# Gwzwpxz/HDSDP

Hardware: AMD Instinct MI355X
Metric: IPM iterations/sec (Schur build+factor+solve), n=2000 m=2000 dense SDP (higher is better)
Workload: dtype f64

## Files before the change

hdsdp_amd/build.py:

```python
import os
import shutil
import subprocess
import sys

PKG = os.path.dirname(os.path.abspath(__file__))
ROOT = os.path.dirname(PKG)
CSRC = os.path.join(PKG, "csrc")
LIB = os.path.join(PKG, "libhdsdp_mi355x.so")
SOURCES = ["gemm_f64.hip", "gemm_persist.hip", "chol.hip", "schur.hip", "lanczos.hip", "lu.hip", "small.hip", "bsparse.hip", "engine.hip", "probes.hip", "coeff.cpp", "sdpa.cpp", "alloc.cpp"]
HEADERS = sorted(f for f in os.listdir(CSRC) if f.endswith(".h")) + [os.path.join(ROOT, "include", "hdsdp_mi355x.h")]


def _stale(target, deps):
    if not os.path.exists(target):
        return True
    t = os.path.getmtime(target)
    return any(os.path.getmtime(d) > t for d in deps)


def build_library(force=False, verbose=True, diagnostics=False):
    srcs = [os.path.join(CSRC, s) for s in SOURCES]
    hdrs = [h if os.path.isabs(h) else os.path.join(CSRC, h) for h in HEADERS]
    lib = LIB.replace(".so", "_diag.so") if diagnostics else LIB
    if not force and not _stale(lib, srcs + hdrs):
# ... 30 lines not shown
```

hdsdp_amd/csrc/gemm_f64.hip:

```cpp
#include "gemm_tile.h"
#include "gemm_persist.h"
namespace {
struct TimedLaunch { hipEvent_t e0, e1; int role; double flops, issued; };
bool g_timing = false;
thread_local bool g_capturing = false;
std::vector<TimedLaunch> g_timed;
unsigned long long *g_dbg = nullptr;
int g_dbg_role = -1;
struct TileList {
    int2 *dev = nullptr;
    int n = 0;
};
std::mutex g_tl_mutex;
std::map<std::tuple<int, int, int, int, int, unsigned long long>, TileList> g_tl_cache;

int g_reserved_cus = 0;
struct PersistDev { int *ring = nullptr; unsigned seq = 0; int slots = 0; };
std::map<int, PersistDev> g_persist_dev;
constexpr int PERSIST_RING = 256;
int persist_counters(int **cnt, int *slots) {
    int dev = 0;
    HDM_HIP_CHECK(hipGetDevice(&dev));
    std::lock_guard<std::mutex> lk(g_tl_mutex);
    PersistDev &pd = g_persist_dev[dev];
// ... 23 lines not shown
    }
    std::vector<int2> h;
    for (const HdmTile &t : hdm_tile_list(gm, subset)) h.push_back(make_int2(t.tm, t.tn));
    TileList tl;
    tl.n = (int) h.size();
    HDM_HIP_CHECK(hdm_malloc((void **) &tl.dev, sizeof(int2) * std::max<size_t>(1, h.size())));
    HDM_HIP_CHECK(hdm_memcpy_h2d_sync(tl.dev, h.data(), sizeof(int2) * h.size()));
    g_tl_cache[key] = tl;
    out = tl;
    return 0;
}
}

static int launch_tiles(const HdmGemmArgs &args, int subset, hipStream_t stream);

static HdmTileGeom tile_geom(const HdmGemmArgs &a) {
    return {a.M, a.N, a.K, a.klimit, a.lower_only, a.tile_col_mask, a.role, a.epilogue == HDM_EPI_SLAB, a.batch, a.k_base, a.k_chunk,
            ((a.role == HDM_ROLE_CONG2 || a.role == HDM_ROLE_GENERIC) && a.A2) ? 2 : 1};
}

static double issued_mfma_flops(const HdmGemmArgs &a, int subset) {
    return (double) hdm_launch_mfmas(tile_geom(a), subset) * 2048.0 * ((a.epilogue == HDM_EPI_SLAB) ? 1.0 : (double) a.batch);
}

int hdm_launch_gemm(const HdmGemmArgs &args, hipStream_t stream) {
    if (args.M <= 0 || args.N <= 0 || args.batch <= 0) return 0;
    if ((args.M % 8) || (args.N % 8) || (args.K % HDM_BK)) {
        fprintf(stderr, "[hdsdp_mi355x] gemm: M,N must be multiples of 8 and K of 16 (M=%d N=%d K=%d)\n",
                args.M, args.N, args.K);
        return 1;
    }
    if (args.epilogue == HDM_EPI_SLAB && (args.k_chunk <= 0 || args.k_chunk % HDM_BK)) {
        fprintf(stderr, "[hdsdp_mi355x] gemm: bad k_chunk\n");
        return 1;
    }
    if (args.role == HDM_ROLE_CONG2) {
        const bool mirrored = args.A2 == args.B && args.B2 == args.A && args.lda2 == args.ldb && args.ldb2 == args.lda &&
                              args.strideA2 == args.strideB && args.strideB2 == args.strideA;
        if (!mirrored || !args.lower_only || args.epilogue != HDM_EPI_BLOCKED || args.klimit != HDM_KLIM_BY_N ||
            args.M != args.N || args.a_kmajor || args.b_kmajor) {
            fprintf(stderr, "[hdsdp_mi355x] gemm role 2 is lower(A B^T + B A^T), blocked output, K cut by the column tile: launch refused\n");
            return 1;
        }
    }
    if (args.role != HDM_ROLE_GENERIC) {
        const long lds_[4] = {args.lda, args.ldb, args.A2 ? args.lda2 : 0, args.B2 ? args.ldb2 : 0};
        for (long ld : lds_)
            if (ld < 0 || ld > (1L << 20)) {
                fprintf(stderr, "[hdsdp_mi355x] gemm role %d: leading dimension %ld is beyond what the scalar stager addresses: launch refused\n", args.role, ld);
                return 1;
            }
        const HdmTileGeom gm = tile_geom(args);
        struct { const double *p; long span; bool km; long ld, kblk, stride; int rows; const char *nm; } ops[4] = {
            {args.A, args.spanA, args.a_kmajor != 0, args.lda, args.a_kblk, args.strideA, args.M, "A"},
            {args.B, args.spanB, args.b_kmajor != 0, args.ldb, args.b_kblk, args.strideB, args.N, "B"},
            {args.A2, args.spanA2, args.a_kmajor != 0, args.lda2, (long) HDM_BK, args.strideA2, args.M, "A2"},
// ... 35 lines not shown
    if (d.dbg && !g_capturing && getenv("HDM_DBG_SYNC")) HDM_HIP_CHECK(hipDeviceSynchronize());
#endif
    int var = 64;
#ifdef HDM_DIAGNOSTICS
    static const int g_env_var = [] { const char *e = getenv("HDM_VAR"); return e ? atoi(e) : -1; }();
    if (g_env_var >= 0) var = g_env_var;
    if (var == 576 && args.role != HDM_ROLE_CONG2) var = 64;
    if (args.role == HDM_ROLE_CONG2) {
        static const int g_direct = [] { const char *e = getenv("HDM_CONG2_DIRECT"); return e ? atoi(e) : 0; }();
        const bool direct = g_direct && var == 64 && args.A2 && !args.a_kmajor && !args.b_kmajor &&
                            args.epilogue == HDM_EPI_BLOCKED && args.lower_only && args.klimit == HDM_KLIM_BY_N &&
                            args.A2 == args.B && args.B2 == args.A;
        if (direct) var = 320;
    }
#endif
    long nwg = (long) tl.n * (args.batch >= 8 ? ((args.batch + 7) & ~7) : args.batch);
    static const int g_persist = [] { const char *e = getenv("HDM_PERSIST"); return e ? atoi(e) : 1; }();
    int *cnt = nullptr;
    const bool persist = g_persist && args.role != HDM_ROLE_GENERIC && args.batch >= 8 && !g_capturing &&
                         hdm_persist_supported(args.a_kmajor != 0, args.b_kmajor != 0, args.role, var);
    if (!persist && (var == 320 || var == 576)) var = 64;
    if (persist) {
        int slots = 0;
        if (persist_counters(&cnt, &slots)) return 1;
        HDM_HIP_CHECK(hipMemsetAsync(cnt, 0, 8 * sizeof(int), stream));
        nwg = std::min<long>(nwg, slots);
    }
    dim3 grid((unsigned) nwg), block(256);
    hipEvent_t e0 = nullptr, e1 = nullptr;
    const bool timed = g_timing && !g_capturing;
// ... 7 lines not shown
    } else {
#define HDM_LAUNCH(AK, BK, R, V) hipLaunchKernelGGL((hdm_gemm_kernel<AK, BK, R, V>), grid, block, 0, stream, d)
#ifdef HDM_DIAGNOSTICS
#define HDM_LAUNCH_V(AK, BK, R)                                   \
    switch (var) {                                                \
        case 32: HDM_LAUNCH(AK, BK, R, 32); break;                \
        case 96: HDM_LAUNCH(AK, BK, R, 96); break;                \
        case 192: HDM_LAUNCH(AK, BK, R, 192); break;              \
        case 0: HDM_LAUNCH(AK, BK, R, 0); break;                  \
        default: HDM_LAUNCH(AK, BK, R, 64);                       \
    }
#else
#define HDM_LAUNCH_V(AK, BK, R) HDM_LAUNCH(AK, BK, R, 64)
#endif
        switch (args.role) {
            case HDM_ROLE_CONG1: HDM_LAUNCH_V(false, true, HDM_ROLE_CONG1); break;
            case HDM_ROLE_CONG2: HDM_LAUNCH_V(false, false, HDM_ROLE_CONG2); break;
            case HDM_ROLE_GRAM: HDM_LAUNCH_V(true, true, HDM_ROLE_GRAM); break;
            case HDM_ROLE_CONG2D: HDM_LAUNCH_V(false, false, HDM_ROLE_CONG2D); break;
            default:
                if (lay == 3) HDM_LAUNCH(true, true, HDM_ROLE_GENERIC, 0);
                else if (lay == 2) HDM_LAUNCH(true, false, HDM_ROLE_GENERIC, 0);
                else if (lay == 1) HDM_LAUNCH(false, true, HDM_ROLE_GENERIC, 0);
#ifdef HDM_DIAGNOSTICS
                else if (var == 32) HDM_LAUNCH(false, false, HDM_ROLE_GENERIC, 32);
#endif
                else HDM_LAUNCH(false, false, HDM_ROLE_GENERIC, 0);
        }
    }
#undef HDM_LAUNCH_V
#undef HDM_LAUNCH
    if (timed) {
// ... 33 lines not shown
```

hdsdp_amd/csrc/gemm_geom.h:

```cpp
#pragma once
#include <algorithm>
#include <utility>
#include <vector>

#if defined(__HIPCC__)
#define HDM_HD __host__ __device__ __attribute__((always_inline))
#else
#define HDM_HD
#endif

#define HDM_TILE 128
#define HDM_BK 16
#define HDM_SUB 16

enum HdmKLimit { HDM_KLIM_NONE = 0, HDM_KLIM_BY_M = 1, HDM_KLIM_BY_N = 2, HDM_KLIM_BAND = 3 };
enum HdmEpilogue {
    HDM_EPI_STORE = 0,
    HDM_EPI_BLOCKED = 1,
    HDM_EPI_SLAB = 2
};
enum HdmRole { HDM_ROLE_GENERIC = 0, HDM_ROLE_CONG1 = 1, HDM_ROLE_CONG2 = 2, HDM_ROLE_GRAM = 3, HDM_ROLE_CONG2D = 4, HDM_NROLES = 5 };

HDM_HD inline long hdm_sky_panel(int t, int n) { return 128L * ((long) t * n - 64L * t * (t - 1)); }
HDM_HD inline long hdm_sky_off(int i, int j, int n) {
// ... 4 lines not shown
    const int t = (n + 127) / 128 - 1;
    const long w = n - 128L * t;
    return hdm_sky_panel(t, n) + w * w;
}

struct HdmTileGeom {
    int M, N, K;
    int klimit;
    int lower_only;
    unsigned long long colmask;
    int role;
    int slab;
    int batch;
    long k_base, k_chunk;
    int npass;
};
struct HdmTile { int tm, tn; };
struct HdmKRange { long kbeg, kend; };

HDM_HD constexpr int hdm_ntiles(int x) { return (x + HDM_TILE - 1) / HDM_TILE; }
HDM_HD constexpr int hdm_valid_subrows(int M, int tm) { return (M - tm * HDM_TILE + 15) >> 4; }
HDM_HD constexpr int hdm_cell_rows(int rv) { return rv < 4 ? 4 : rv; }
HDM_HD constexpr bool hdm_colmask_honoured(int NT) { return NT <= 64; }
HDM_HD constexpr unsigned long long hdm_colmask_effective(unsigned long long mask, int NT) { return hdm_colmask_honoured(NT) ? mask : 0ULL; }

HDM_HD constexpr bool hdm_tile_selected(const HdmTileGeom &g, int tm, int tn) {
    const unsigned long long mask = hdm_colmask_effective(g.colmask, hdm_ntiles(g.N));
    return !((g.lower_only || g.klimit == HDM_KLIM_BAND) && tm < tn) && !(mask && !((mask >> tn) & 1ULL));
}
HDM_HD constexpr bool hdm_full_diag(int M, int tm, int tn) { return tm == tn && hdm_valid_subrows(M, tm) >= 8; }
// ... 66 lines not shown
constexpr HdmLive HDM_LIVE_CONG1_FIRST[HDM_KBLOCK_PAIRS] = {{0, 0, 0}, {0, 1, 0}, {0, 2, 0}, {0, 3, 0}};
constexpr HdmLive HDM_LIVE_CONG1_LAST[HDM_KBLOCK_PAIRS] = {{0, 3, 0}, {0, 3, 1}, {0, 3, 2}, {0, 3, 3}};

HDM_HD constexpr int hdm_live_per_kstep(HdmLive l) { return (l.jhi - l.jlo + 1) * (4 - l.ilo); }
HDM_HD constexpr long hdm_pair_mfmas(HdmLive l) { return 2L * 4 * 4 * hdm_live_per_kstep(l); }
constexpr long HDM_KBLOCK_MFMAS = HDM_KBLOCK_PAIRS * hdm_pair_mfmas(HDM_LIVE_FULL);
HDM_HD constexpr long hdm_block_mfmas(const HdmLive (&t)[HDM_KBLOCK_PAIRS]) {
    long s = 0;
    for (int p = 0; p < HDM_KBLOCK_PAIRS; ++p) s += hdm_pair_mfmas(t[p]);
    return s;
}
HDM_HD constexpr long hdm_even_stages(long nst) { return nst <= 0 ? 0 : ((nst + 1) / 2) * 2; }
constexpr int HDM_DIAG_CELLS = 36;
HDM_HD constexpr int hdm_diag_short_cells(int RV) { return RV * (RV + 1) / 2; }
HDM_HD constexpr int hdm_edge_cells(int RV) { return 8 * RV; }
HDM_HD constexpr long hdm_tile_mfmas(const HdmTileGeom &g, int tm, int tn, int z) {
    const long nst = hdm_tile_stages(g, tm, tn, z);
    if (g.role == HDM_ROLE_GENERIC) return hdm_pair_mfmas(HDM_LIVE_FULL) / 2 * nst;
    const HdmTileClass c = hdm_tile_class(g, tm, tn);
    switch (c.kind) {
        case HDM_CLS_DIAG_FULL: return 4L * HDM_DIAG_CELLS * hdm_even_stages(nst);
        case HDM_CLS_DIAG_SHORT: return 4L * hdm_diag_short_cells(c.RV) * hdm_even_stages(nst);
        case HDM_CLS_EDGE: return 4L * hdm_edge_cells(c.RV) * hdm_even_stages(nst);
        case HDM_CLS_SYMDIAG: return tn * HDM_KBLOCK_MFMAS + hdm_block_mfmas(HDM_LIVE_CONG2D_LAST);
        default: break;
    }
    if (g.role == HDM_ROLE_CONG2) return 2 * (tn * HDM_KBLOCK_MFMAS + hdm_block_mfmas(HDM_LIVE_CONG2_LAST));
    if (g.role == HDM_ROLE_CONG1)
        return hdm_block_mfmas(HDM_LIVE_CONG1_FIRST) + (tm - tn - 1) * HDM_KBLOCK_MFMAS + hdm_block_mfmas(HDM_LIVE_CONG1_LAST);
    return hdm_pair_mfmas(HDM_LIVE_FULL) / 2 * hdm_even_stages(nst);
}
inline long hdm_launch_mfmas(const HdmTileGeom &g, int subset) {
    long mf = 0;
    for (int z = 0; z < (g.slab ? g.batch : 1); ++z)
// ... 68 lines not shown
```

hdsdp_amd/csrc/gemm_persist.h:

```cpp
#pragma once
#include "gemm_tile.h"

bool hdm_persist_supported(bool a_kmajor, bool b_kmajor, int role, int variant);
int hdm_launch_persist(bool a_kmajor, bool b_kmajor, int role, int variant, dim3 grid, dim3 block, hipStream_t stream,
                       const HdmGemmDev &d, int *cnt);
```

hdsdp_amd/csrc/gemm_persist.hip:

```cpp
#include "gemm_persist.h"

template <bool AK, bool BK, int R, int V>
static int launch_p(dim3 grid, dim3 block, hipStream_t stream, const HdmGemmDev &d, int *cnt) {
    hipLaunchKernelGGL((hdm_gemm_persist_kernel<AK, BK, R, V>), grid, block, 0, stream, d, cnt);
    return 0;
}

bool hdm_persist_supported(bool a_kmajor, bool b_kmajor, int role, int variant) {
#ifdef HDM_DIAGNOSTICS
    const bool common = (variant == 64 || variant == 96 || variant == 192);
    const bool cong2_extra = (variant == 320 || variant == 576);
#else
    const bool common = (variant == 64), cong2_extra = false;
#endif
    if (role == HDM_ROLE_CONG1) return !a_kmajor && b_kmajor && common;
    if (role == HDM_ROLE_CONG2) return !a_kmajor && !b_kmajor && (common || cong2_extra);
    if (role == HDM_ROLE_GRAM) return a_kmajor && b_kmajor && common;
    if (role == HDM_ROLE_CONG2D) return !a_kmajor && !b_kmajor && common;
    return false;
}

int hdm_launch_persist(bool a_kmajor, bool b_kmajor, int role, int variant, dim3 grid, dim3 block, hipStream_t stream,
                       const HdmGemmDev &d, int *cnt) {
    if (role == HDM_ROLE_CONG1 && !a_kmajor && b_kmajor) {
        if (variant == 64) return launch_p<false, true, HDM_ROLE_CONG1, 64>(grid, block, stream, d, cnt);
#ifdef HDM_DIAGNOSTICS
        if (variant == 96) return launch_p<false, true, HDM_ROLE_CONG1, 96>(grid, block, stream, d, cnt);
        if (variant == 192) return launch_p<false, true, HDM_ROLE_CONG1, 192>(grid, block, stream, d, cnt);
#endif
    } else if (role == HDM_ROLE_CONG2 && !a_kmajor && !b_kmajor) {
        if (variant == 64) return launch_p<false, false, HDM_ROLE_CONG2, 64>(grid, block, stream, d, cnt);
#ifdef HDM_DIAGNOSTICS
        if (variant == 96) return launch_p<false, false, HDM_ROLE_CONG2, 96>(grid, block, stream, d, cnt);
        if (variant == 192) return launch_p<false, false, HDM_ROLE_CONG2, 192>(grid, block, stream, d, cnt);
        if (variant == 320) return launch_p<false, false, HDM_ROLE_CONG2, 320>(grid, block, stream, d, cnt);
        if (variant == 576) return launch_p<false, false, HDM_ROLE_CONG2, 576>(grid, block, stream, d, cnt);
#endif
    } else if (role == HDM_ROLE_CONG2D && !a_kmajor && !b_kmajor) {
        if (variant == 64) return launch_p<false, false, HDM_ROLE_CONG2D, 64>(grid, block, stream, d, cnt);
#ifdef HDM_DIAGNOSTICS
        if (variant == 96) return launch_p<false, false, HDM_ROLE_CONG2D, 96>(grid, block, stream, d, cnt);
        if (variant == 192) return launch_p<false, false, HDM_ROLE_CONG2D, 192>(grid, block, stream, d, cnt);
#endif
    } else if (role == HDM_ROLE_GRAM && a_kmajor && b_kmajor) {
        if (variant == 64) return launch_p<true, true, HDM_ROLE_GRAM, 64>(grid, block, stream, d, cnt);
// ... 10 lines not shown
```

hdsdp_amd/csrc/gemm_tile.h:

```cpp
#pragma once
#include "hdm_common.h"
#include <algorithm>
#include <map>
#include <mutex>
#include <tuple>
#include <vector>

#define LDM 144
#define LDK 18
#define STAGE_DOUBLES 2304

struct HdmGemmDev {
    HdmGemmArgs a;
    const int2 *tiles;
    int ntiles;
    unsigned long long *dbg;
};

template <bool KM, bool DUAL = true>
struct Stager {
    const double *p;
    long qstride;
    long kstep;
    unsigned okmask;
// ... 244 lines not shown

template <class T> constexpr bool cell_uses_row(int q) {
    for (int c = 0; c < T::NC; ++c) if (T::si[c] == q) return true;
    return false;
}
template <class T> constexpr bool cell_uses_col(int q) {
    for (int c = 0; c < T::NC; ++c) if (T::sj[c] == q) return true;
    return false;
}
template <class T> constexpr int cell_frag_count() {
    int k = 0;
    for (int q = 0; q < 8; ++q) k += (cell_uses_row<T>(q) ? 1 : 0) + (cell_uses_col<T>(q) ? 1 : 0);
    return k;
}

template <class T, bool AKM, bool BKM, class STA, class STB>
__device__ __forceinline__ void cell_tile(const HdmGemmArgs &a, STA &stA, STB &stB, hdm_lchar *sb,
                                          int nst, int tid, int z, int m0, int n0, int l15, int lq, int rv, int tri) {
    hdm_d4 acc[4][4];
#pragma unroll
    for (int c = 0; c < 16; ++c) acc[c >> 2][c & 3] = (hdm_d4){0.0, 0.0, 0.0, 0.0};
    hdm_u4 ra0, ra1, ra2, ra3, rb0, rb1, rb2, rb3;
    double fr0[8], fc0[8], fr1[8], fc1[8];
    constexpr int NC = T::NC;
    constexpr int NF = cell_frag_count<T>();
    const hdm_lchar *rdA = sb + rd_lane<AKM>(0, l15, lq);
    const hdm_lchar *rdB = sb + 2 * STAGE_DOUBLES * 8 + rd_lane<BKM>(0, l15, lq);
    hdm_lchar *wrA = sb + wr_lane<AKM>(tid);
    hdm_lchar *wrB = sb + 2 * STAGE_DOUBLES * 8 + wr_lane<BKM>(tid);
#define HDM_CLDF(FR, FC, CB, kk)                                                                            \
    _Pragma("unroll") for (int q = 0; q < 8; ++q) {                                                         \
        if (cell_uses_row<T>(q)) FR[q] = lds_ld(rdA + rd_off<AKM>(CB, q, kk));                              \
        if (cell_uses_col<T>(q)) FC[q] = lds_ld(rdB + rd_off<BKM>(CB, q, kk));                              \
    }
#define HDM_CMMA(FR, FC)                                                                                    \
    _Pragma("unroll") for (int c = 0; c < NC; ++c)                                                          \
        acc[c >> 2][c & 3] = __builtin_amdgcn_mfma_f64_16x16x4f64(FC[T::sj[c]], FR[T::si[c]], acc[c >> 2][c & 3], 0, 0, 0);
#define HDM_CSTAGE(CB)                                                                                      \
    {                                                                                                       \
        HDM_CLDF(fr1, fc1, CB, 4)                                                                           \
        HDM_CMMA(fr0, fc0)                                                                                  \
        HDM_CLDF(fr0, fc0, CB, 8)                                                                           \
        HDM_CMMA(fr1, fc1)                                                                                  \
        HDM_CLDF(fr1, fc1, CB, 12)                                                                          \
        st4(wrA, (CB) ^ 1, ra0, ra1, ra2, ra3); st4(wrB, (CB) ^ 1, rb0, rb1, rb2, rb3);                     \
        HDM_CMMA(fr0, fc0)                                                                                  \
        sgb_spread<NC, 0x100, NF>();                                                                        \
        sgb_spread<NC, 0x100, NF>();                                                                        \
        sgb_spread<NC / 2, 0x100, NF>();                                                                    \
        sgb_spread<NC - NC / 2, 0x200, 8>();                                                                \
        __builtin_amdgcn_sched_barrier(0);                                                                  \
        __syncthreads();                                                                                    \
        __builtin_amdgcn_sched_barrier(0);                                                                  \
        HDM_CLDF(fr0, fc0, (CB) ^ 1, 0)                                                                     \
        stA.load_counted(ra0, ra1, ra2, ra3); stB.load_counted(rb0, rb1, rb2, rb3);    \
        HDM_CMMA(fr1, fc1)                                                                                  \
        __builtin_amdgcn_sched_group_barrier(0x100, NF, 0);                                                 \
        sgb_spread<NC, 0x20, 8>();                                                                          \
        __builtin_amdgcn_sched_barrier(0);                                                                  \
    }
#define HDM_CLAST(CB)                                                                                       \
    {                                                                                                       \
        HDM_CLDF(fr1, fc1, CB, 4)                                                                           \
        HDM_CMMA(fr0, fc0)                                                                                  \
        HDM_CLDF(fr0, fc0, CB, 8)                                                                           \
        HDM_CMMA(fr1, fc1)                                                                                  \
        HDM_CLDF(fr1, fc1, CB, 12)                                                                          \
        HDM_CMMA(fr0, fc0)                                                                                  \
        HDM_CMMA(fr1, fc1)                                                                                  \
    }
    stA.remain = nst; stB.remain = nst;
    if (nst > 0) {
        stA.load_counted(ra0, ra1, ra2, ra3); stB.load_counted(rb0, rb1, rb2, rb3);
        st4(wrA, 0, ra0, ra1, ra2, ra3); st4(wrB, 0, rb0, rb1, rb2, rb3);
        stA.load_counted(ra0, ra1, ra2, ra3); stB.load_counted(rb0, rb1, rb2, rb3);
    }
    __syncthreads();
    if (nst > 0) {
        HDM_CLDF(fr0, fc0, 0, 0)
        const int npairs = (nst + 1) >> 1;
        for (int t = 0; t + 1 < npairs; ++t) { HDM_CSTAGE(0) HDM_CSTAGE(1) }
        HDM_CSTAGE(0) HDM_CLAST(1)
    }
#undef HDM_CLDF
#undef HDM_CMMA
#undef HDM_CSTAGE
#undef HDM_CLAST
    cell_epilogue<T>(a, z, m0, n0, l15, lq, rv, tri, acc);
}

template <int JLO>
__device__ __forceinline__ void cd_mma(hdm_d4 (&acc)[4][4], const double (&fa)[4], const double (&fb)[4]) {
#pragma unroll
    for (int j = JLO; j < 4; ++j)
#pragma unroll
        for (int i = 0; i < 4; ++i) acc[j][i] = __builtin_amdgcn_mfma_f64_16x16x4f64(fa[j], fb[i], acc[j][i], 0, 0, 0);
}

// ... 108 lines not shown

    const int kt0 = (int) (kbeg / HDM_BK), kt1 = (int) (kend / HDM_BK);
    constexpr bool symdiag = (ROLE == HDM_ROLE_CONG2D);
#define HDM_CELL_STAMP(KIND)                                                                        \
    if ((VAR & 32) && p.dbg && tid == 0) {                                                          \
        unsigned long long *d = p.dbg + (size_t) sidx * 8;                                    \
        d[0] = t_start; d[1] = t_start; d[2] = t_start; d[3] = __builtin_amdgcn_s_memtime();        \
        d[4] = __builtin_amdgcn_s_getreg((15 << 11) | (0 << 6) | 4);                                \
        d[5] = __builtin_amdgcn_s_getreg((3 << 11) | (0 << 6) | 20);                                \
        d[6] = (unsigned long long) (long long) -(KIND);                                            \
        d[7] = __builtin_amdgcn_s_memrealtime();                                                    \
    }

    if constexpr (ROLE != HDM_ROLE_GENERIC) {
    constexpr bool DUAL = (ROLE == HDM_ROLE_CONG2);
    SStager<AKM, DUAL> stA;
    SStager<BKM, DUAL> stB;
    long ldb = a.ldb;
    if (ROLE == HDM_ROLE_CONG1 && a.b_sky) {
        ldb = a.N - 128L * tn;
        B += hdm_sky_panel(tn, a.N) - 128L * tn * (ldb + 1);
    }
    stA.init(A, a.lda, a.a_kblk, a.seg_rows, a.seg_extra, (VAR & 128) ? 0 : m0, kt0, tid, wave);
    stB.init(B, ldb, a.b_kblk, a.seg_rows, a.seg_extra, (VAR & 128) ? 0 : n0, kt0, tid, wave);
    int npass = 1;
    if constexpr (DUAL) {
        if (a.A2) {
            npass = 2;
            stA.chain(a.A2 + (long) z * a.strideA2, a.lda2, m0, kt0, wave, kt1 - kt0);
            stB.chain(a.B2 + (long) z * a.strideB2, a.ldb2, n0, kt0, wave, kt1 - kt0);
        }
    }
    if (!symdiag && a.lower_only && tm == tn) {
        const int nst = (kt1 - kt0) * npass;
        const int rvd = (a.M - m0 + 15) >> 4;
        if (rvd < 8) {
#define HDM_DEDGE(RV)                                                                                                      \
    switch (wave) {                                                                                                        \
        case 0: cell_tile<DiagEdgeCells<0, RV>, AKM, BKM>(a, stA, stB, sb, nst, tid, z, m0, n0, l15, lq, rvd, 1); break;  \
        case 1: cell_tile<DiagEdgeCells<1, RV>, AKM, BKM>(a, stA, stB, sb, nst, tid, z, m0, n0, l15, lq, rvd, 1); break;  \
        case 2: cell_tile<DiagEdgeCells<2, RV>, AKM, BKM>(a, stA, stB, sb, nst, tid, z, m0, n0, l15, lq, rvd, 1); break;  \
        default: cell_tile<DiagEdgeCells<3, RV>, AKM, BKM>(a, stA, stB, sb, nst, tid, z, m0, n0, l15, lq, rvd, 1); break; \
    }
            if (rvd <= 4) { HDM_DEDGE(4) } else if (rvd == 5) { HDM_DEDGE(5) } else if (rvd == 6) { HDM_DEDGE(6) } else { HDM_DEDGE(7) }
#undef HDM_DEDGE
            HDM_CELL_STAMP(3)
            return;
        }
        if constexpr (ROLE != HDM_ROLE_CONG2) {
            switch (wave) {
                case 0: cell_tile<DiagCells<0>, AKM, BKM>(a, stA, stB, sb, nst, tid, z, m0, n0, l15, lq, 8, 1); break;
                case 1: cell_tile<DiagCells<1>, AKM, BKM>(a, stA, stB, sb, nst, tid, z, m0, n0, l15, lq, 8, 1); break;
                case 2: cell_tile<DiagCells<2>, AKM, BKM>(a, stA, stB, sb, nst, tid, z, m0, n0, l15, lq, 8, 1); break;
                default: cell_tile<DiagCells<3>, AKM, BKM>(a, stA, stB, sb, nst, tid, z, m0, n0, l15, lq, 8, 1); break;
            }
            HDM_CELL_STAMP(1)
        }
        return;
    }
    if (!symdiag && tm != tn && m0 + HDM_TILE > a.M && n0 + HDM_TILE <= a.N) {
        const int nst = (kt1 - kt0) * npass;
        const int rv = (a.M - m0 + 15) >> 4;
#define HDM_EDGE(RV)                                                                                                     \
    switch (wave) {                                                                                                      \
        case 0: cell_tile<EdgeCells<0, RV>, AKM, BKM>(a, stA, stB, sb, nst, tid, z, m0, n0, l15, lq, rv, 0); break;  \
        case 1: cell_tile<EdgeCells<1, RV>, AKM, BKM>(a, stA, stB, sb, nst, tid, z, m0, n0, l15, lq, rv, 0); break;  \
        case 2: cell_tile<EdgeCells<2, RV>, AKM, BKM>(a, stA, stB, sb, nst, tid, z, m0, n0, l15, lq, rv, 0); break;  \
        default: cell_tile<EdgeCells<3, RV>, AKM, BKM>(a, stA, stB, sb, nst, tid, z, m0, n0, l15, lq, rv, 0); break; \
    }
        if (rv <= 4) { HDM_EDGE(4) } else if (rv == 5) { HDM_EDGE(5) } else if (rv == 6) { HDM_EDGE(6) } else { HDM_EDGE(7) }
#undef HDM_EDGE
        HDM_CELL_STAMP(2)
        return;
    }

    if constexpr (ROLE == HDM_ROLE_CONG2 && (VAR & 256) != 0) {
        cong2_direct_body(a, z, tm, tn, wm, wn, l15, lq);
        return;
    }
    {
        hdm_u4 ra0, ra1, ra2, ra3, rb0, rb1, rb2, rb3;
        const int nst = (kt1 - kt0) * npass;
        double fa0[4], fb0[4], fa1[4], fb1[4];
        const hdm_lchar *rdA = sb + rd_lane<AKM>(wm * 16, l15, lq);
        const hdm_lchar *rdB = sb + 2 * STAGE_DOUBLES * 8 + rd_lane<BKM>(wn * 16, l15, lq);
        hdm_lchar *wrA = sb + wr_lane<AKM>(tid);
        hdm_lchar *wrB = sb + 2 * STAGE_DOUBLES * 8 + wr_lane<BKM>(tid);
#define HDM_LDF(FA, FB, CB, kk)                                                                   \
    _Pragma("unroll") for (int i = 0; i < 4; ++i) FB[i] = lds_ld(rdA + rd_off<AKM>(CB, 2 * i, kk)); \
// ... 295 lines not shown
    const int x = (int) __builtin_amdgcn_s_getreg((3 << 11) | (0 << 6) | 20) & 7;
    const bool one_queue = (ROLE == HDM_ROLE_GRAM) && p.a.queue_global != 0;
    for (int dx = 0; dx < (one_queue ? 1 : 8); ++dx) {
        const int xq = one_queue ? 0 : ((x + dx) & 7);
        while (true) {
            __syncthreads();
            if (threadIdx.x == 0) s_idx = atomicAdd(&cnt[xq], 1);
            __syncthreads();
            const int idx = __builtin_amdgcn_readfirstlane(s_idx);
            const int z = one_queue ? idx / ntiles : xq + 8 * (idx / ntiles);
            if (z >= nb) break;
            hdm_gemm_tile<AKM, BKM, ROLE, VAR>(p, z, idx % ntiles, (long) z * ntiles + idx % ntiles);
        }
    }
}
```

Baseline: 2.858.

## Skip dead MFMA cells per K stage in CONG1/CONG2 diagonal and edge tiles

Adds an exact-liveness mode, on by default through HDM_EXACT_LIVE, for the CONG1 and CONG2 roles. Diagonal and edge cell tiles unroll their first and last K blocks with compile-time masks, so MFMAs whose sub-tile contributes only zeros at a given stage are not issued. The CONG2 edge path also uses unmasked loads. The old pair-live path is kept as a separate kernel variant in a new source file for when the mode is turned off. This trims wasted matrix-core work on triangular and banded tiles, at the cost of more template instantiations, larger code, and possible register pressure.

New measurement: 2.870 (median of 6 runs). Within noise of the previous version (+0.4%).

```diff
diff --git a/hdsdp_amd/build.py b/hdsdp_amd/build.py
--- a/hdsdp_amd/build.py
+++ b/hdsdp_amd/build.py
@@ -7,7 +7,7 @@
 ROOT = os.path.dirname(PKG)
 CSRC = os.path.join(PKG, "csrc")
 LIB = os.path.join(PKG, "libhdsdp_mi355x.so")
-SOURCES = ["gemm_f64.hip", "gemm_persist.hip", "chol.hip", "schur.hip", "lanczos.hip", "lu.hip", "small.hip", "bsparse.hip", "engine.hip", "probes.hip", "coeff.cpp", "sdpa.cpp", "alloc.cpp"]
+SOURCES = ["gemm_f64.hip", "gemm_persist.hip", "gemm_pairlive.hip", "chol.hip", "schur.hip", "lanczos.hip", "lu.hip", "small.hip", "bsparse.hip", "engine.hip", "probes.hip", "coeff.cpp", "sdpa.cpp", "alloc.cpp"]
 HEADERS = sorted(f for f in os.listdir(CSRC) if f.endswith(".h")) + [os.path.join(ROOT, "include", "hdsdp_mi355x.h")]
 
 
diff --git a/hdsdp_amd/csrc/gemm_f64.hip b/hdsdp_amd/csrc/gemm_f64.hip
--- a/hdsdp_amd/csrc/gemm_f64.hip
+++ b/hdsdp_amd/csrc/gemm_f64.hip
@@ -61,9 +61,15 @@
 
 static int launch_tiles(const HdmGemmArgs &args, int subset, hipStream_t stream);
 
+static bool exact_live() {
+    static const int g_exact = [] { const char *e = getenv("HDM_EXACT_LIVE"); return e ? atoi(e) : 1; }();
+    return g_exact != 0;
+}
+
 static HdmTileGeom tile_geom(const HdmGemmArgs &a) {
     return {a.M, a.N, a.K, a.klimit, a.lower_only, a.tile_col_mask, a.role, a.epilogue == HDM_EPI_SLAB, a.batch, a.k_base, a.k_chunk,
-            ((a.role == HDM_ROLE_CONG2 || a.role == HDM_ROLE_GENERIC) && a.A2) ? 2 : 1};
+            ((a.role == HDM_ROLE_CONG2 || a.role == HDM_ROLE_GENERIC) && a.A2) ? 2 : 1,
+            ((a.role == HDM_ROLE_CONG1 || a.role == HDM_ROLE_CONG2) && exact_live()) ? (HDM_EXACT_CELLS | HDM_EXACT_CELLS2) : 0};
 }
 
 static double issued_mfma_flops(const HdmGemmArgs &a, int subset) {
@@ -87,6 +93,13 @@
         if (!mirrored || !args.lower_only || args.epilogue != HDM_EPI_BLOCKED || args.klimit != HDM_KLIM_BY_N ||
             args.M != args.N || args.a_kmajor || args.b_kmajor) {
             fprintf(stderr, "[hdsdp_mi355x] gemm role 2 is lower(A B^T + B A^T), blocked output, K cut by the column tile: launch refused\n");
+            return 1;
+        }
+    }
+    if (args.role == HDM_ROLE_CONG1) {
+        if (args.klimit != HDM_KLIM_BAND || !args.lower_only || args.M != args.N || args.M != args.K || args.epilogue == HDM_EPI_SLAB ||
+            args.a_kmajor || !args.b_kmajor || args.A2 || args.B2) {
+            fprintf(stderr, "[hdsdp_mi355x] gemm role 1 is lower(A B^T) over the K band of a square launch, A M-major, B K-major: launch refused\n");
             return 1;
         }
     }
@@ -152,6 +165,7 @@
         if (direct) var = 320;
     }
 #endif
+    if (var == 64 && !exact_live() && (args.role == HDM_ROLE_CONG1 || args.role == HDM_ROLE_CONG2)) var = 64 | HDM_VAR_PAIR_LIVE;
     long nwg = (long) tl.n * (args.batch >= 8 ? ((args.batch + 7) & ~7) : args.batch);
     static const int g_persist = [] { const char *e = getenv("HDM_PERSIST"); return e ? atoi(e) : 1; }();
     int *cnt = nullptr;
@@ -189,8 +203,14 @@
 #define HDM_LAUNCH_V(AK, BK, R) HDM_LAUNCH(AK, BK, R, 64)
 #endif
         switch (args.role) {
-            case HDM_ROLE_CONG1: HDM_LAUNCH_V(false, true, HDM_ROLE_CONG1); break;
-            case HDM_ROLE_CONG2: HDM_LAUNCH_V(false, false, HDM_ROLE_CONG2); break;
+            case HDM_ROLE_CONG1:
+                if (var == (64 | HDM_VAR_PAIR_LIVE)) { if (hdm_launch_pairlive(args.role, grid, block, stream, d, nullptr)) return 1; }
+                else HDM_LAUNCH_V(false, true, HDM_ROLE_CONG1);
+                break;
+            case HDM_ROLE_CONG2:
+                if (var == (64 | HDM_VAR_PAIR_LIVE)) { if (hdm_launch_pairlive(args.role, grid, block, stream, d, nullptr)) return 1; }
+                else HDM_LAUNCH_V(false, false, HDM_ROLE_CONG2);
+                break;
             case HDM_ROLE_GRAM: HDM_LAUNCH_V(true, true, HDM_ROLE_GRAM); break;
             case HDM_ROLE_CONG2D: HDM_LAUNCH_V(false, false, HDM_ROLE_CONG2D); break;
             default:
diff --git a/hdsdp_amd/csrc/gemm_geom.h b/hdsdp_amd/csrc/gemm_geom.h
--- a/hdsdp_amd/csrc/gemm_geom.h
+++ b/hdsdp_amd/csrc/gemm_geom.h
@@ -42,6 +42,7 @@
     int batch;
     long k_base, k_chunk;
     int npass;
+    int exact_live;
 };
 struct HdmTile { int tm, tn; };
 struct HdmKRange { long kbeg, kend; };
@@ -138,10 +139,85 @@
 constexpr int HDM_DIAG_CELLS = 36;
 HDM_HD constexpr int hdm_diag_short_cells(int RV) { return RV * (RV + 1) / 2; }
 HDM_HD constexpr int hdm_edge_cells(int RV) { return 8 * RV; }
+
+enum HdmZeroRule {
+    HDM_Z_NONE = 0,
+    HDM_Z_COLS_UPTO = 1,
+    HDM_Z_ROWS_FROM = 2,
+    HDM_Z_COLS_FROM = 4
+};
+constexpr int HDM_Z_CONG1_FIRST = HDM_Z_COLS_UPTO, HDM_Z_CONG1_LAST = HDM_Z_ROWS_FROM;
+constexpr int HDM_Z_CONG1_DIAG = HDM_Z_COLS_UPTO | HDM_Z_ROWS_FROM;
+constexpr int HDM_Z_CONG2_LAST = HDM_Z_COLS_FROM;
+constexpr int HDM_Z_CONG2D_LAST = HDM_Z_ROWS_FROM | HDM_Z_COLS_FROM;
+constexpr int HDM_KBLOCK_STAGES = HDM_TILE / HDM_BK;
+HDM_HD constexpr bool hdm_subtile_live(int rules, int s, int si, int sj) {
+    return !((rules & HDM_Z_COLS_UPTO) && sj > s) && !((rules & HDM_Z_ROWS_FROM) && si < s) && !((rules & HDM_Z_COLS_FROM) && sj < s);
+}
+HDM_HD constexpr HdmLive hdm_live_exact(int rules, int s, int wm, int wn) {
+    return {(rules & HDM_Z_COLS_FROM) ? (s - wn + 1) / 2 : 0, (rules & HDM_Z_COLS_UPTO) ? (s - wn + 2) / 2 - 1 : 3,
+            (rules & HDM_Z_ROWS_FROM) ? (s - wm + 1) / 2 : 0};
+}
+HDM_HD constexpr long hdm_block_mfmas_exact(int rules) {
+    long mf = 0;
+    for (int s = 0; s < HDM_KBLOCK_STAGES; ++s)
+        for (int w = 0; w < 4; ++w) mf += 4L * hdm_live_per_kstep(hdm_live_exact(rules, s, w & 1, w >> 1));
+    return mf;
+}
+struct HdmStageRange { int lo, hi; };
+HDM_HD constexpr HdmStageRange hdm_cell_stage_range(int rules, int si, int sj) {
+    const int hi_r = (rules & HDM_Z_ROWS_FROM) ? si : HDM_KBLOCK_STAGES - 1, hi_c = (rules & HDM_Z_COLS_FROM) ? sj : HDM_KBLOCK_STAGES - 1;
+    return {(rules & HDM_Z_COLS_UPTO) ? sj : 0, hi_r < hi_c ? hi_r : hi_c};
+}
+HDM_HD constexpr int hdm_cells_live(HdmTileKind kind, int RV, int rules, int s) {
+    int n = 0;
+    for (int si = 0; si < (kind == HDM_CLS_DIAG_FULL ? 8 : RV); ++si)
+        for (int sj = 0; sj < (kind == HDM_CLS_EDGE ? 8 : si + 1); ++sj) {
+            const HdmStageRange r = hdm_cell_stage_range(rules, si, sj);
+            n += (r.lo <= s && s <= r.hi) ? 1 : 0;
+        }
+    return n;
+}
+HDM_HD constexpr long hdm_cell_block_mfmas(HdmTileKind kind, int RV, int rules, int nstages) {
+    long mf = 0;
+    for (int s = 0; s < nstages; ++s) mf += 4L * hdm_cells_live(kind, RV, rules, s);
+    return mf;
+}
+enum HdmExactLive { HDM_EXACT_CELLS = 1, HDM_EXACT_MAIN = 2, HDM_EXACT_CELLS2 = 4 };
+HDM_HD constexpr int hdm_exact_stages(int RV) { return RV >= 8 ? 8 : (RV + 1) / 2 * 2; }
+HDM_HD constexpr long hdm_tile_mfmas_exact(const HdmTileGeom &g, const HdmTileClass &c, int tm, int tn) {
+    const bool cells = (g.exact_live & HDM_EXACT_CELLS) != 0, mains = (g.exact_live & HDM_EXACT_MAIN) != 0;
+    if (g.role == HDM_ROLE_CONG1) {
+        if (c.kind == HDM_CLS_DIAG_FULL || c.kind == HDM_CLS_DIAG_SHORT)
+            return cells ? hdm_cell_block_mfmas(c.kind, c.RV, HDM_Z_CONG1_DIAG, c.RV) : -1;
+        if (c.kind == HDM_CLS_EDGE)
+            return cells ? hdm_cell_block_mfmas(c.kind, c.RV, HDM_Z_CONG1_FIRST, HDM_KBLOCK_STAGES) +
+                               (tm - tn - 1) * 4L * hdm_edge_cells(c.RV) * HDM_KBLOCK_STAGES +
+                               hdm_cell_block_mfmas(c.kind, c.RV, HDM_Z_CONG1_LAST, c.RV)
+                         : -1;
+        return mains ? hdm_block_mfmas_exact(HDM_Z_CONG1_FIRST) + (tm - tn - 1) * HDM_KBLOCK_MFMAS + hdm_block_mfmas_exact(HDM_Z_CONG1_LAST) : -1;
+    }
+    if (g.role == HDM_ROLE_CONG2) {
+        if (c.kind == HDM_CLS_EDGE)
+            return (g.exact_live & HDM_EXACT_CELLS2) ? 2 * (tn * 4L * hdm_edge_cells(c.RV) * HDM_KBLOCK_STAGES +
+                                hdm_cell_block_mfmas(c.kind, c.RV, HDM_Z_CONG2_LAST, HDM_KBLOCK_STAGES))
+                         : -1;
+        if (c.kind == HDM_CLS_MAIN) return mains ? 2 * (tn * HDM_KBLOCK_MFMAS + hdm_block_mfmas_exact(HDM_Z_CONG2_LAST)) : -1;
+        return -1;
+    }
+    if (g.role == HDM_ROLE_CONG2D && c.kind == HDM_CLS_SYMDIAG)
+        return mains ? tn * HDM_KBLOCK_MFMAS + hdm_block_mfmas_exact(HDM_Z_CONG2D_LAST) : -1;
+    return -1;
+}
+
 HDM_HD constexpr long hdm_tile_mfmas(const HdmTileGeom &g, int tm, int tn, int z) {
     const long nst = hdm_tile_stages(g, tm, tn, z);
     if (g.role == HDM_ROLE_GENERIC) return hdm_pair_mfmas(HDM_LIVE_FULL) / 2 * nst;
     const HdmTileClass c = hdm_tile_class(g, tm, tn);
+    if (g.exact_live) {
+        const long mf = hdm_tile_mfmas_exact(g, c, tm, tn);
+        if (mf >= 0) return mf;
+    }
     switch (c.kind) {
         case HDM_CLS_DIAG_FULL: return 4L * HDM_DIAG_CELLS * hdm_even_stages(nst);
         case HDM_CLS_DIAG_SHORT: return 4L * hdm_diag_short_cells(c.RV) * hdm_even_stages(nst);
diff --git a/hdsdp_amd/csrc/gemm_pairlive.hip b/hdsdp_amd/csrc/gemm_pairlive.hip
--- /dev/null
+++ b/hdsdp_amd/csrc/gemm_pairlive.hip
@@ -0,0 +1,16 @@
+#include "gemm_persist.h"
+
+int hdm_launch_pairlive(int role, dim3 grid, dim3 block, hipStream_t stream, const HdmGemmDev &d, int *cnt) {
+    constexpr int V = 64 | HDM_VAR_PAIR_LIVE;
+    if (role == HDM_ROLE_CONG1) {
+        if (cnt) hipLaunchKernelGGL((hdm_gemm_pairlive_kernel<false, true, HDM_ROLE_CONG1>), grid, block, 0, stream, d, cnt);
+        else hipLaunchKernelGGL((hdm_gemm_kernel<false, true, HDM_ROLE_CONG1, V>), grid, block, 0, stream, d);
+        return 0;
+    }
+    if (role == HDM_ROLE_CONG2) {
+        if (cnt) hipLaunchKernelGGL((hdm_gemm_pairlive_kernel<false, false, HDM_ROLE_CONG2>), grid, block, 0, stream, d, cnt);
+        else hipLaunchKernelGGL((hdm_gemm_kernel<false, false, HDM_ROLE_CONG2, V>), grid, block, 0, stream, d);
+        return 0;
+    }
+    return 1;
+}
diff --git a/hdsdp_amd/csrc/gemm_persist.h b/hdsdp_amd/csrc/gemm_persist.h
--- a/hdsdp_amd/csrc/gemm_persist.h
+++ b/hdsdp_amd/csrc/gemm_persist.h
@@ -4,3 +4,4 @@
 bool hdm_persist_supported(bool a_kmajor, bool b_kmajor, int role, int variant);
 int hdm_launch_persist(bool a_kmajor, bool b_kmajor, int role, int variant, dim3 grid, dim3 block, hipStream_t stream,
                        const HdmGemmDev &d, int *cnt);
+int hdm_launch_pairlive(int role, dim3 grid, dim3 block, hipStream_t stream, const HdmGemmDev &d, int *cnt);
diff --git a/hdsdp_amd/csrc/gemm_persist.hip b/hdsdp_amd/csrc/gemm_persist.hip
--- a/hdsdp_amd/csrc/gemm_persist.hip
+++ b/hdsdp_amd/csrc/gemm_persist.hip
@@ -7,6 +7,7 @@
 }
 
 bool hdm_persist_supported(bool a_kmajor, bool b_kmajor, int role, int variant) {
+    if (variant == (64 | HDM_VAR_PAIR_LIVE)) return (role == HDM_ROLE_CONG1 && !a_kmajor && b_kmajor) || (role == HDM_ROLE_CONG2 && !a_kmajor && !b_kmajor);
 #ifdef HDM_DIAGNOSTICS
     const bool common = (variant == 64 || variant == 96 || variant == 192);
     const bool cong2_extra = (variant == 320 || variant == 576);
@@ -23,12 +24,14 @@
 int hdm_launch_persist(bool a_kmajor, bool b_kmajor, int role, int variant, dim3 grid, dim3 block, hipStream_t stream,
                        const HdmGemmDev &d, int *cnt) {
     if (role == HDM_ROLE_CONG1 && !a_kmajor && b_kmajor) {
+        if (variant == (64 | HDM_VAR_PAIR_LIVE)) return hdm_launch_pairlive(role, grid, block, stream, d, cnt);
         if (variant == 64) return launch_p<false, true, HDM_ROLE_CONG1, 64>(grid, block, stream, d, cnt);
 #ifdef HDM_DIAGNOSTICS
         if (variant == 96) return launch_p<false, true, HDM_ROLE_CONG1, 96>(grid, block, stream, d, cnt);
         if (variant == 192) return launch_p<false, true, HDM_ROLE_CONG1, 192>(grid, block, stream, d, cnt);
 #endif
     } else if (role == HDM_ROLE_CONG2 && !a_kmajor && !b_kmajor) {
+        if (variant == (64 | HDM_VAR_PAIR_LIVE)) return hdm_launch_pairlive(role, grid, block, stream, d, cnt);
         if (variant == 64) return launch_p<false, false, HDM_ROLE_CONG2, 64>(grid, block, stream, d, cnt);
 #ifdef HDM_DIAGNOSTICS
         if (variant == 96) return launch_p<false, false, HDM_ROLE_CONG2, 96>(grid, block, stream, d, cnt);
diff --git a/hdsdp_amd/csrc/gemm_tile.h b/hdsdp_amd/csrc/gemm_tile.h
--- a/hdsdp_amd/csrc/gemm_tile.h
+++ b/hdsdp_amd/csrc/gemm_tile.h
@@ -6,6 +6,7 @@
 #include <tuple>
 #include <vector>
 
+#define HDM_VAR_PAIR_LIVE 1024
 #define LDM 144
 #define LDK 18
 #define STAGE_DOUBLES 2304
@@ -282,7 +283,15 @@
     return k;
 }
 
-template <class T, bool AKM, bool BKM, class STA, class STB>
+enum { HDM_XM_LOOP = 0, HDM_XM_CONG1_DIAG = 1, HDM_XM_CONG1_EDGE = 2, HDM_XM_CONG2_EDGE = 3 };
+template <class T> constexpr bool cellx_live(int rules, int s, int c) { return hdm_subtile_live(rules, s, T::si[c], T::sj[c]); }
+template <class T> constexpr int cellx_cells(int rules, int s) {
+    int k = 0;
+    for (int c = 0; c < T::NC; ++c) k += cellx_live<T>(rules, s, c) ? 1 : 0;
+    return k;
+}
+
+template <class T, bool AKM, bool BKM, int XM = HDM_XM_LOOP, int NS = 8, class STA, class STB>
 __device__ __forceinline__ void cell_tile(const HdmGemmArgs &a, STA &stA, STB &stB, hdm_lchar *sb,
                                           int nst, int tid, int z, int m0, int n0, int l15, int lq, int rv, int tri) {
     hdm_d4 acc[4][4];
@@ -296,6 +305,9 @@
     const hdm_lchar *rdB = sb + 2 * STAGE_DOUBLES * 8 + rd_lane<BKM>(0, l15, lq);
     hdm_lchar *wrA = sb + wr_lane<AKM>(tid);
     hdm_lchar *wrB = sb + 2 * STAGE_DOUBLES * 8 + wr_lane<BKM>(tid);
+#define HDM_STLOAD                                                                                          \
+    if constexpr (XM == HDM_XM_CONG2_EDGE) { stA.load_nomask(ra0, ra1, ra2, ra3); stB.load_nomask(rb0, rb1, rb2, rb3); }       \
+    else { stA.load_counted(ra0, ra1, ra2, ra3); stB.load_counted(rb0, rb1, rb2, rb3); }
 #define HDM_CLDF(FR, FC, CB, kk)                                                                            \
     _Pragma("unroll") for (int q = 0; q < 8; ++q) {                                                         \
         if (cell_uses_row<T>(q)) FR[q] = lds_ld(rdA + rd_off<AKM>(CB, q, kk));                              \
@@ -321,7 +333,7 @@
         __syncthreads();                                                                                    \
         __builtin_amdgcn_sched_barrier(0);                                                                  \
         HDM_CLDF(fr0, fc0, (CB) ^ 1, 0)                                                                     \
-        stA.load_counted(ra0, ra1, ra2, ra3); stB.load_counted(rb0, rb1, rb2, rb3);    \
+        HDM_STLOAD    \
         HDM_CMMA(fr1, fc1)                                                                                  \
         __builtin_amdgcn_sched_group_barrier(0x100, NF, 0);                                                 \
         sgb_spread<NC, 0x20, 8>();                                                                          \
@@ -337,19 +349,97 @@
         HDM_CMMA(fr0, fc0)                                                                                  \
         HDM_CMMA(fr1, fc1)                                                                                  \
     }
+#define HDM_XMMA(FR, FC, Z, S)                                                                              \
+    _Pragma("unroll") for (int c = 0; c < NC; ++c)                                                          \
+        if (cellx_live<T>(Z, S, c))                                                                         \
+            acc[c >> 2][c & 3] = __builtin_amdgcn_mfma_f64_16x16x4f64(FC[T::sj[c]], FR[T::si[c]], acc[c >> 2][c & 3], 0, 0, 0);
+#define HDM_XSTAGE_(CB, Z, S, SW)                                                                              \
+    {                                                                                                       \
+        constexpr int NL = cellx_cells<T>(Z, S);                                 \
+        HDM_CLDF(fr1, fc1, CB, 4)                                                                           \
+        HDM_XMMA(fr0, fc0, Z, S)                                                                            \
+        HDM_CLDF(fr0, fc0, CB, 8)                                                                           \
+        HDM_XMMA(fr1, fc1, Z, S)                                                                            \
+        HDM_CLDF(fr1, fc1, CB, 12)                                                                          \
+        st4(wrA, (CB) ^ 1, ra0, ra1, ra2, ra3); st4(wrB, (CB) ^ 1, rb0, rb1, rb2, rb3);                     \
+        HDM_XMMA(fr0, fc0, Z, S)                                                                            \
+        sgb_spread<NL, 0x100, NF>();                                                                        \
+        sgb_spread<NL, 0x100, NF>();                                                                        \
+        sgb_spread<NL / 2, 0x100, NF>();                                                                    \
+        sgb_spread<NL - NL / 2, 0x200, 8>();                                                                \
+        __builtin_amdgcn_sched_barrier(0);                                                                  \
+        __syncthreads();                                                                                    \
+        __builtin_amdgcn_sched_barrier(0);                                                                  \
+        HDM_CLDF(fr0, fc0, (CB) ^ 1, 0)                                                                     \
+        HDM_STLOAD    \
+        if constexpr (SW) { stA.second(); stB.second(); }    \
+        HDM_XMMA(fr1, fc1, Z, S)                                                                            \
+        __builtin_amdgcn_sched_group_barrier(0x100, NF, 0);                                                 \
+        sgb_spread<NL, 0x20, 8>();                                                                          \
+        __builtin_amdgcn_sched_barrier(0);                                                                  \
+    }
+#define HDM_XSTAGE(CB, Z, S) HDM_XSTAGE_(CB, Z, S, false)
+#define HDM_XLAST(CB, Z, S)                                                                                 \
+    {                                                                                                       \
+        HDM_CLDF(fr1, fc1, CB, 4)                                                                           \
+        HDM_XMMA(fr0, fc0, Z, S)                                                                            \
+        HDM_CLDF(fr0, fc0, CB, 8)                                                                           \
+        HDM_XMMA(fr1, fc1, Z, S)                                                                            \
+        HDM_CLDF(fr1, fc1, CB, 12)                                                                          \
+        HDM_XMMA(fr0, fc0, Z, S)                                                                            \
+        HDM_XMMA(fr1, fc1, Z, S)                                                                            \
+    }
+#define HDM_XBLOCK8(Z)                                                                                      \
+    HDM_XSTAGE(0, Z, 0) HDM_XSTAGE(1, Z, 1) HDM_XSTAGE(0, Z, 2) HDM_XSTAGE(1, Z, 3)                         \
+    HDM_XSTAGE(0, Z, 4) HDM_XSTAGE(1, Z, 5) HDM_XSTAGE(0, Z, 6) HDM_XSTAGE(1, Z, 7)
+#define HDM_XBLOCK8SW(Z)                                                                                    \
+    HDM_XSTAGE(0, Z, 0) HDM_XSTAGE(1, Z, 1) HDM_XSTAGE(0, Z, 2) HDM_XSTAGE(1, Z, 3)                         \
+    HDM_XSTAGE(0, Z, 4) HDM_XSTAGE_(1, Z, 5, true) HDM_XSTAGE(0, Z, 6) HDM_XSTAGE(1, Z, 7)
+#define HDM_XEND(Z, NE)                                                                                     \
+    HDM_XSTAGE(0, Z, 0) HDM_XSTAGE(1, Z, 1) HDM_XSTAGE(0, Z, 2)                                             \
+    if constexpr ((NE) == 4) { HDM_XLAST(1, Z, 3) } else {                                                  \
+        HDM_XSTAGE(1, Z, 3) HDM_XSTAGE(0, Z, 4)                                                             \
+        if constexpr ((NE) == 6) { HDM_XLAST(1, Z, 5) } else {                                              \
+            HDM_XSTAGE(1, Z, 5) HDM_XSTAGE(0, Z, 6) HDM_XLAST(1, Z, 7)                                      \
+        }                                                                                                   \
+    }
+#define HDM_XFULL2 { HDM_CSTAGE(0) HDM_CSTAGE(1) }
+    static_assert(NS == 4 || NS == 6 || NS == 8, "a last block runs 4, 6 or 8 stages");
     stA.remain = nst; stB.remain = nst;
     if (nst > 0) {
-        stA.load_counted(ra0, ra1, ra2, ra3); stB.load_counted(rb0, rb1, rb2, rb3);
+        HDM_STLOAD
         st4(wrA, 0, ra0, ra1, ra2, ra3); st4(wrB, 0, rb0, rb1, rb2, rb3);
-        stA.load_counted(ra0, ra1, ra2, ra3); stB.load_counted(rb0, rb1, rb2, rb3);
+        HDM_STLOAD
     }
     __syncthreads();
     if (nst > 0) {
         HDM_CLDF(fr0, fc0, 0, 0)
-        const int npairs = (nst + 1) >> 1;
-        for (int t = 0; t + 1 < npairs; ++t) { HDM_CSTAGE(0) HDM_CSTAGE(1) }
-        HDM_CSTAGE(0) HDM_CLAST(1)
-    }
+        if constexpr (XM == HDM_XM_CONG1_DIAG) {
+            HDM_XEND(HDM_Z_CONG1_DIAG, NS)
+        } else if constexpr (XM == HDM_XM_CONG1_EDGE) {
+            HDM_XBLOCK8(HDM_Z_CONG1_FIRST)
+            for (int t = 0; t < ((nst - rv) >> 1) - HDM_KBLOCK_PAIRS; ++t) HDM_XFULL2
+            HDM_XEND(HDM_Z_CONG1_LAST, NS)
+        } else if constexpr (XM == HDM_XM_CONG2_EDGE) {
+            for (int t = 0; t < (nst >> 2) - HDM_KBLOCK_PAIRS; ++t) HDM_XFULL2
+            HDM_XBLOCK8SW(HDM_Z_CONG2_LAST)
+            for (int t = 0; t < (nst >> 2) - HDM_KBLOCK_PAIRS; ++t) HDM_XFULL2
+            HDM_XEND(HDM_Z_CONG2_LAST, 8)
+        } else {
+            const int npairs = (nst + 1) >> 1;
+            for (int t = 0; t + 1 < npairs; ++t) { HDM_CSTAGE(0) HDM_CSTAGE(1) }
+            HDM_CSTAGE(0) HDM_CLAST(1)
+        }
+    }
+#undef HDM_XFULL2
+#undef HDM_XEND
+#undef HDM_XBLOCK8
+#undef HDM_XLAST
+#undef HDM_XSTAGE
+#undef HDM_XSTAGE_
+#undef HDM_XBLOCK8SW
+#undef HDM_STLOAD
+#undef HDM_XMMA
 #undef HDM_CLDF
 #undef HDM_CMMA
 #undef HDM_CSTAGE
@@ -488,6 +578,10 @@
 
     if constexpr (ROLE != HDM_ROLE_GENERIC) {
     constexpr bool DUAL = (ROLE == HDM_ROLE_CONG2);
+    constexpr bool XLIVE = (VAR & HDM_VAR_PAIR_LIVE) == 0;
+    constexpr int XDIAG = (XLIVE && ROLE == HDM_ROLE_CONG1) ? HDM_XM_CONG1_DIAG : HDM_XM_LOOP;
+    constexpr int XEDGE = !XLIVE ? HDM_XM_LOOP : ROLE == HDM_ROLE_CONG1 ? HDM_XM_CONG1_EDGE : ROLE == HDM_ROLE_CONG2 ? HDM_XM_CONG2_EDGE : HDM_XM_LOOP;
+#define HDM_CELL_BRANCH(c) ((ROLE == HDM_ROLE_CONG1 && XLIVE) ? __builtin_expect((c), 0) : (c))
     SStager<AKM, DUAL> stA;
     SStager<BKM, DUAL> stB;
     long ldb = a.ldb;
@@ -505,16 +599,16 @@
             stB.chain(a.B2 + (long) z * a.strideB2, a.ldb2, n0, kt0, wave, kt1 - kt0);
         }
     }
-    if (!symdiag && a.lower_only && tm == tn) {
+    if (HDM_CELL_BRANCH(!symdiag && a.lower_only && tm == tn)) {
         const int nst = (kt1 - kt0) * npass;
         const int rvd = (a.M - m0 + 15) >> 4;
         if (rvd < 8) {
 #define HDM_DEDGE(RV)                                                                                                      \
     switch (wave) {                                                                                                        \
-        case 0: cell_tile<DiagEdgeCells<0, RV>, AKM, BKM>(a, stA, stB, sb, nst, tid, z, m0, n0, l15, lq, rvd, 1); break;  \
-        case 1: cell_tile<DiagEdgeCells<1, RV>, AKM, BKM>(a, stA, stB, sb, nst, tid, z, m0, n0, l15, lq, rvd, 1); break;  \
-        case 2: cell_tile<DiagEdgeCells<2, RV>, AKM, BKM>(a, stA, stB, sb, nst, tid, z, m0, n0, l15, lq, rvd, 1); break;  \
-        default: cell_tile<DiagEdgeCells<3, RV>, AKM, BKM>(a, stA, stB, sb, nst, tid, z, m0, n0, l15, lq, rvd, 1); break; \
+        case 0: cell_tile<DiagEdgeCells<0, RV>, AKM, BKM, XDIAG, hdm_exact_stages(RV)>(a, stA, stB, sb, nst, tid, z, m0, n0, l15, lq, rvd, 1); break;  \
+        case 1: cell_tile<DiagEdgeCells<1, RV>, AKM, BKM, XDIAG, hdm_exact_stages(RV)>(a, stA, stB, sb, nst, tid, z, m0, n0, l15, lq, rvd, 1); break;  \
+        case 2: cell_tile<DiagEdgeCells<2, RV>, AKM, BKM, XDIAG, hdm_exact_stages(RV)>(a, stA, stB, sb, nst, tid, z, m0, n0, l15, lq, rvd, 1); break;  \
+        default: cell_tile<DiagEdgeCells<3, RV>, AKM, BKM, XDIAG, hdm_exact_stages(RV)>(a, stA, stB, sb, nst, tid, z, m0, n0, l15, lq, rvd, 1); break; \
     }
             if (rvd <= 4) { HDM_DEDGE(4) } else if (rvd == 5) { HDM_DEDGE(5) } else if (rvd == 6) { HDM_DEDGE(6) } else { HDM_DEDGE(7) }
 #undef HDM_DEDGE
@@ -523,30 +617,31 @@
         }
         if constexpr (ROLE != HDM_ROLE_CONG2) {
             switch (wave) {
-                case 0: cell_tile<DiagCells<0>, AKM, BKM>(a, stA, stB, sb, nst, tid, z, m0, n0, l15, lq, 8, 1); break;
-                case 1: cell_tile<DiagCells<1>, AKM, BKM>(a, stA, stB, sb, nst, tid, z, m0, n0, l15, lq, 8, 1); break;
-                case 2: cell_tile<DiagCells<2>, AKM, BKM>(a, stA, stB, sb, nst, tid, z, m0, n0, l15, lq, 8, 1); break;
-                default: cell_tile<DiagCells<3>, AKM, BKM>(a, stA, stB, sb, nst, tid, z, m0, n0, l15, lq, 8, 1); break;
+                case 0: cell_tile<DiagCells<0>, AKM, BKM, XDIAG, 8>(a, stA, stB, sb, nst, tid, z, m0, n0, l15, lq, 8, 1); break;
+                case 1: cell_tile<DiagCells<1>, AKM, BKM, XDIAG, 8>(a, stA, stB, sb, nst, tid, z, m0, n0, l15, lq, 8, 1); break;
+                case 2: cell_tile<DiagCells<2>, AKM, BKM, XDIAG, 8>(a, stA, stB, sb, nst, tid, z, m0, n0, l15, lq, 8, 1); break;
+                default: cell_tile<DiagCells<3>, AKM, BKM, XDIAG, 8>(a, stA, stB, sb, nst, tid, z, m0, n0, l15, lq, 8, 1); break;
             }
             HDM_CELL_STAMP(1)
         }
         return;
     }
-    if (!symdiag && tm != tn && m0 + HDM_TILE > a.M && n0 + HDM_TILE <= a.N) {
+    if (HDM_CELL_BRANCH(!symdiag && tm != tn && m0 + HDM_TILE > a.M && n0 + HDM_TILE <= a.N)) {
         const int nst = (kt1 - kt0) * npass;
         const int rv = (a.M - m0 + 15) >> 4;
 #define HDM_EDGE(RV)                                                                                                     \
     switch (wave) {                                                                                                      \
-        case 0: cell_tile<EdgeCells<0, RV>, AKM, BKM>(a, stA, stB, sb, nst, tid, z, m0, n0, l15, lq, rv, 0); break;  \
-        case 1: cell_tile<EdgeCells<1, RV>, AKM, BKM>(a, stA, stB, sb, nst, tid, z, m0, n0, l15, lq, rv, 0); break;  \
-        case 2: cell_tile<EdgeCells<2, RV>, AKM, BKM>(a, stA, stB, sb, nst, tid, z, m0, n0, l15, lq, rv, 0); break;  \
-        default: cell_tile<EdgeCells<3, RV>, AKM, BKM>(a, stA, stB, sb, nst, tid, z, m0, n0, l15, lq, rv, 0); break; \
+        case 0: cell_tile<EdgeCells<0, RV>, AKM, BKM, XEDGE, XEDGE == HDM_XM_CONG1_EDGE ? hdm_exact_stages(RV) : 8>(a, stA, stB, sb, nst, tid, z, m0, n0, l15, lq, rv, 0); break;  \
+        case 1: cell_tile<EdgeCells<1, RV>, AKM, BKM, XEDGE, XEDGE == HDM_XM_CONG1_EDGE ? hdm_exact_stages(RV) : 8>(a, stA, stB, sb, nst, tid, z, m0, n0, l15, lq, rv, 0); break;  \
+        case 2: cell_tile<EdgeCells<2, RV>, AKM, BKM, XEDGE, XEDGE == HDM_XM_CONG1_EDGE ? hdm_exact_stages(RV) : 8>(a, stA, stB, sb, nst, tid, z, m0, n0, l15, lq, rv, 0); break;  \
+        default: cell_tile<EdgeCells<3, RV>, AKM, BKM, XEDGE, XEDGE == HDM_XM_CONG1_EDGE ? hdm_exact_stages(RV) : 8>(a, stA, stB, sb, nst, tid, z, m0, n0, l15, lq, rv, 0); break; \
     }
         if (rv <= 4) { HDM_EDGE(4) } else if (rv == 5) { HDM_EDGE(5) } else if (rv == 6) { HDM_EDGE(6) } else { HDM_EDGE(7) }
 #undef HDM_EDGE
         HDM_CELL_STAMP(2)
         return;
     }
+#undef HDM_CELL_BRANCH
 
     if constexpr (ROLE == HDM_ROLE_CONG2 && (VAR & 256) != 0) {
         cong2_direct_body(a, z, tm, tn, wm, wn, l15, lq);
@@ -872,3 +967,23 @@
         }
     }
 }
+
+template <bool AKM, bool BKM, int ROLE>
+__global__ __launch_bounds__(256, 2) void hdm_gemm_pairlive_kernel(HdmGemmDev p, int *__restrict__ cnt) {
+    __shared__ int s_idx;
+    const int nb = p.a.batch, ntiles = p.ntiles;
+    const int x = (int) __builtin_amdgcn_s_getreg((3 << 11) | (0 << 6) | 20) & 7;
+    const bool one_queue = (ROLE == HDM_ROLE_GRAM) && p.a.queue_global != 0;
+    for (int dx = 0; dx < (one_queue ? 1 : 8); ++dx) {
+        const int xq = one_queue ? 0 : ((x + dx) & 7);
+        while (true) {
+            __syncthreads();
+            if (threadIdx.x == 0) s_idx = atomicAdd(&cnt[xq], 1);
+            __syncthreads();
+            const int idx = __builtin_amdgcn_readfirstlane(s_idx);
+            const int z = one_queue ? idx / ntiles : xq + 8 * (idx / ntiles);
+            if (z >= nb) break;
+            hdm_gemm_tile<AKM, BKM, ROLE, 64 | HDM_VAR_PAIR_LIVE>(p, z, idx % ntiles, (long) z * ntiles + idx % ntiles);
+        }
+    }
+}
```
